# ruc-aimc-lab/LAFF

Hardware: AMD Instinct MI355X
Metric: text-video cosine pairs/sec (higher is better)
Workload: dtype f32 towers (FC on fp16 hi/lo split x3 MFMA) + fp16 similarity

## Files before the change

### laff_amd/build.py

```python
import os
import subprocess
import sys
from concurrent.futures import ThreadPoolExecutor

HERE = os.path.dirname(os.path.abspath(__file__))
CSRC = os.path.join(HERE, 'csrc')
LIBDIR = os.path.join(HERE, 'lib')
LIB = os.path.join(LIBDIR, 'liblaff_hip.so')
SOURCES = ['gemm_nt.hip', 'sim_strip.hip', 'fc_strip.hip', 'fc_concat.hip', 'fuse.hip', 'fuse_bwd.hip', 'frame_bwd.hip', 'fc_bwd.hip', 'optim.hip', 'rank.hip', 'loss.hip', 'loss_dsl.hip', 'gru.hip', 'clip.hip', 'clip_image.hip', 'frame_prep.hip', 'bert.hip', 'netvlad.hip', 'rerank.hip', 'sim_hist.hip', 'comm.hip', 'api.hip']
HEADERS = [os.path.join(CSRC, 'kernels.h'), os.path.join(CSRC, 'clip_core.h'), os.path.join(CSRC, 'exact_cos.h'), os.path.join(CSRC, 'strip_util.h'), os.path.join(CSRC, 'wave_reduce.h'), os.path.join(os.path.dirname(HERE), 'include', 'laff_hip.h')]
ARCH = 'gfx950'
FLAGS = ['-O3', '-std=c++20', '-fPIC', '--offload-arch=' + ARCH, '-fno-gpu-rdc', '-Wall', '-Wno-unused-function']


def hipcc():
    for c in (os.environ.get('HIPCC'), '/opt/rocm/bin/hipcc', 'hipcc'):
        if c and (os.path.isabs(c) and os.path.exists(c) or not os.path.isabs(c)):
            return c
    raise RuntimeError('hipcc not found')


def _stale(target, deps):
    if not os.path.exists(target):
        return True
# ... 43 lines not shown
```

### laff_amd/csrc/api.hip

```cpp
#include <hip/hip_runtime.h>

#include <algorithm>
#include <climits>
#include <cmath>
#include <cstdarg>
#include <cstdio>
#include <cstdlib>
#include <cstring>
#include <string>
#include <vector>

#include "kernels.h"

constexpr int METRIC_SLOTS = 33;

struct laff_ctx {
    int device;
    hipStream_t stream;
    double* d_metrics = nullptr;
    unsigned metrics_slot = 0;
    double* h_metrics = nullptr;
    char* d_mscratch = nullptr;
};

// ... 115 lines not shown
    return LAFF_OK;
}

}

extern "C" {

int laff_abi_version(void) { return LAFF_ABI_VERSION; }

const char* laff_last_error(void) { return g_err.c_str(); }

int laff_ctx_create(int device, void* hip_stream, laff_ctx** out) {
    if (!out) return fail(LAFF_E_ARG, "laff_ctx_create: null out");
    auto knob = [](const char* name, int dflt) { const char* e = getenv(name); return e ? atoi(e) : dflt; };
    laff::g_strip_mode = knob("LAFF_STRIP", 1);
    int n = 0;
    HIP_TRY(hipGetDeviceCount(&n));
    if (device < 0 || device >= n) return fail(LAFF_E_ARG, "laff_ctx_create: device %d out of range (%d devices)", device, n);
    hipDeviceProp_t prop;
    HIP_TRY(hipGetDeviceProperties(&prop, device));
    if (strncmp(prop.gcnArchName, "gfx950", 6) != 0)
        return fail(LAFF_E_UNSUPPORTED, "laff_ctx_create: device %d is %s; this library is built for gfx950 only", device,
                    prop.gcnArchName);
    if (prop.multiProcessorCount > 0) laff::g_num_cus = prop.multiProcessorCount;
    laff_ctx* c = new laff_ctx();
    c->device = device;
    c->stream = static_cast<hipStream_t>(hip_stream);
    *out = c;
    return LAFF_OK;
}
// ... 2061 lines not shown
```

### laff_amd/csrc/fc_strip.hip

```cpp
#include <hip/hip_runtime.h>
#include <stdint.h>

#include <algorithm>
#include <cstdlib>
#include <vector>

#include "kernels.h"
#include "strip_util.h"

namespace laff {

namespace {

using namespace su;

typedef __attribute__((address_space(1))) unsigned gu32;

constexpr int FR = FC_STRIP_ROWS;
constexpr int SLOT = 32 * 1024;
constexpr int PLANE = 16 * 1024;
constexpr int RING = 4;
constexpr int PIECES = 8;
constexpr int XB_OFF = RING * SLOT;
constexpr int SMEM = XB_OFF + SLOT;
// ... 576 lines not shown
        const float b = bias ? bias[n] : 0.f, g = bn_scale ? bn_scale[n] : 1.f, t = bn_shift ? bn_shift[n] : 0.f;
        float4 c;
        if (act == LAFF_ACT_TANH) c = make_float4(cs * 2.885390081777927f, b * 2.885390081777927f, -2.f * g, g + t);
        else if (act == LAFF_ACT_SIGMOID) c = make_float4(cs * -1.4426950408889634f, b * -1.4426950408889634f, g, t);
        else if (act == LAFF_ACT_RELU) c = make_float4(cs, b, g, t);
        else c = make_float4(cs * g, fmaf(b, g, t), 0.f, 0.f);
        *(float4*)(vec + 4 * (size_t)n) = c;
    }
}

size_t fc_strip_image_bytes(int D) { return (size_t)(D / 32) * (2 * SLOT) + (size_t)D * 16; }
size_t fc_strip_vec_offset(int D) { return (size_t)(D / 32) * (2 * SLOT); }

hipError_t launch_fc_strip_pack(const float* W, int ldw, const float* bias, const float* bn_scale, const float* bn_shift, int D, int act,
                                void* img, hipStream_t st) {
    hipLaunchKernelGGL(fc_strip_pack_kernel, dim3((unsigned)D), dim3(256), 0, st, W, ldw, bias, bn_scale, bn_shift, D, act,
                       (_Float16*)img, (float*)((char*)img + fc_strip_vec_offset(D)));
    return hipGetLastError();
}

hipError_t launch_fc_strip(FcStripArgs& a, int act, hipStream_t st) {
    long U = 0;
    for (int i = 0; i < a.count; ++i) {
        a.p[i].unit0 = (int)U;
        U += (long)((a.p[i].N + FR - 1) / FR) * a.nblk;
    }
    if (U == 0) return hipSuccess;
    if (U >= (1l << 31)) return hipErrorInvalidValue;
    a.total_units = (int)U;
    a.trace = nullptr;
#ifdef LAFF_FCS_TRACE
    if (const char* e = getenv("LAFF_GEMM_TRACE_PTR")) a.trace = (unsigned long long*)strtoull(e, nullptr, 0);
#endif
    const int G = (int)std::min<long>(std::min(g_num_cus, STRIP_MAX_WG), U);
    a.nranges = G;
    for (int b = 0; b < G; ++b) a.range_of_wg[b] = (unsigned short)((G % 8 == 0) ? (b % 8) * (G / 8) + b / 8 : b);
#define LAFF_FCS_LAUNCH(K)                                                                                                    \
    do {                                                                                                                      \
        static unsigned long long attr_done = 0;                                                                              \
        if (hipError_t e = smem_attr_once(attr_done, fc_strip_kernel<K>, SMEM); e != hipSuccess) return e;                    \
        hipLaunchKernelGGL((fc_strip_kernel<K>), dim3((unsigned)G), dim3(256), SMEM, st, a);                                  \
    } while (0)
    if (act == LAFF_ACT_TANH || act == LAFF_ACT_SIGMOID) LAFF_FCS_LAUNCH(ACT_EXP);
    else if (act == LAFF_ACT_RELU) LAFF_FCS_LAUNCH(ACT_RELU);
    else LAFF_FCS_LAUNCH(ACT_LIN);
#undef LAFF_FCS_LAUNCH
    return hipGetLastError();
}

}
```

### laff_amd/csrc/kernels.h

```cpp
#pragma once
#include <hip/hip_runtime.h>
#include <stdint.h>

#include "../../include/laff_hip.h"

namespace laff {

template <typename K>
static inline hipError_t smem_attr_once(unsigned long long& done, K kernel, int smem) {
    int dev = 0;
    hipError_t e = hipGetDevice(&dev);
    if (e != hipSuccess) return e;
    const unsigned long long bit = 1ull << (dev & 63);
    if (__atomic_load_n(&done, __ATOMIC_ACQUIRE) & bit) return hipSuccess;
    if (smem > 64 * 1024) {
        e = hipFuncSetAttribute((const void*)kernel, hipFuncAttributeMaxDynamicSharedMemorySize, smem);
        if (e != hipSuccess) return e;
    }
    __atomic_fetch_or(&done, bit, __ATOMIC_ACQ_REL);
    return hipSuccess;
}

enum { GEMM_F32 = 0, GEMM_F16 = 1, GEMM_BF16 = 2 };

// ... 76 lines not shown
};
struct FcStripArgs {
    int count;
    int nblk;
    int nranges;
    int total_units;
    unsigned long long* trace;
    FcStripProblem p[MAX_GROUP];
    unsigned short range_of_wg[STRIP_MAX_WG];
};
size_t fc_strip_image_bytes(int D);
size_t fc_strip_vec_offset(int D);
hipError_t launch_fc_strip_pack(const float* W, int ldw, const float* bias, const float* bn_scale, const float* bn_shift, int D, int act,
                                void* img, hipStream_t st);
hipError_t launch_fc_strip(FcStripArgs& a, int act, hipStream_t st);

constexpr int CONCAT_MAX_SEG = 8;
constexpr int CONCAT_MAX_GROUP = 4;
struct ConcatDense {
    const float* X;
    int ldx, dk, c0;
    int fast;
};
struct ConcatSparse {
    const int* indptr;
    const int* indices;
    const float* values;
    const float* wt;
    int ldwt, dk;
};
// ... 423 lines not shown
```

### laff_amd/model/model.py

```python
import numpy as np

import torch
import torch.nn as nn
import torch.nn.functional as F

from .. import loss as _loss
from .. import ops
from .Attention import Attention_1, JustAverage, Multi_head_MyApply_Attention

device = torch.device('cuda')
float16 = False
FC_PRECISION = 'fp32'


def _row_chunks(pending, limit_bytes=1 << 31):
    out = []
    for q in pending:
        x = q['x']
        if not torch.is_tensor(x) or x.layout != torch.strided or x.dim() != 2:
            out.append(q)
            continue
        n, k = x.shape
        row_bytes = 4 * max(x.stride(0) if n > 1 else k, (k + 63) // 64 * 64)
        if n * row_bytes < limit_bytes:
# ... 211 lines not shown
        return out

    def weight_split(self):
        if FC_PRECISION != 'fp16x3':
            return None
        w = self.fc1.weight
        key = (w.data_ptr(), w._version)
        if getattr(self, '_w_split', None) is None or self._w_split[0] != key:
            self._w_split = (key, ops.split_rows(w.detach()))
        return self._w_split[1]

    def strip_weights(self):
        scale, shift = self.bn_affine(None)
        w, b = self.fc1.weight, self.fc1.bias
        key = (w.data_ptr(), w._version, None if b is None else (b.data_ptr(), b._version),
               None if self.bn1 is None else self._bn_cache[0], self.activation_name)
        if getattr(self, '_w_strip', None) is None or self._w_strip[0] != key:
            self._w_strip = (key, ops.fc_strip_pack(w.detach(), None if b is None else b.detach(), scale, shift, self.activation_name))
        return self._w_strip[1]

    def _forward_train(self, x, heads=1, extra_shift=None):
        if self.fc1 is None:
            raise NotImplementedError('training mode: a TransformNet without fc (fc=False%s) has no differentiable path; apply its '
                                      'BatchNorm upstream as a torch op' % (', tiled over %d heads' % heads if heads > 1 else ''))
        if x.layout != torch.strided:
            raise NotImplementedError('training mode: a sparse (CSR) input has no backward (laff_fc_gather_act_bn is inference only)')
        if extra_shift is not None:
            raise NotImplementedError('training mode: extra_shift (the expert embedding) is not differentiable here; add it upstream '
                                      'as a torch op')
        y = _FcActFn.apply(x, self.fc1.weight, self.fc1.bias, self.activation_name)
        if self.dropout_p is not None:
# ... 717 lines not shown
```

### laff_amd/ops.py

```python
import ctypes as C

import numpy as np
import torch

from . import _lib
from ._lib import (ACT, GRU_POOLING, ATT_JUST_AVERAGE, ATT_L2NORM_EACH_HEAD, ATT_MUL, ATT_NO_SPLIT_HEAD, ATT_WITH_AVE, PREC,
                   FcProblem, FcSplitProblem, FcStripProblem, Plane, check, FcFusedProblem, RankSide, FcConcatProblem, FcConcatSegment,
                   FcLaunch, FcShape, RerankProblem)

__all__ = ['sim_hist', 'rerank_workspace_bytes', 'rerank_run', 'rerank_tkb', 'frame_preprocess', 'frame_desc_device', 'netvlad_workspace_bytes', 'netvlad_encode', 'bert_workspace_bytes', 'bert_encode', 'clip_pack_weight', 'clip_workspace_bytes', 'clip_encode', 'gru_pack_whh', 'gru_workspace_bytes', 'gru_encode', 'rank_resolve_metrics', 'rank_prepare', 'rank_prepare_text', 'rank_band_video', 'rank_export_pairs', 'rank_resolve_list', 'sim_gemm_banded', 'rank_resolve', 'exact_ranks', 'RankState', 'topk_rows', 'topk_from_operands', 'alloc_scores', 'frame_fuse_grouped', 'fc_act_bn_fused_grouped', 'fused_split_eligible', 'fc_strip_pack', 'fc_strip_eligible', 'fc_act_bn_strip_grouped', 'StripWeights', 'margin_loss', 'dsl_loss', 'margin_loss_scores', 'fc_gather_act_bn', 'fc_act_bn', 'fc_act_bn_grouped', 'fc_act_bn_split_grouped', 'split_rows', 'row_dot_gt', 'rank_metrics_async', 'fuse', 'fuse_backward', 'fc_backward', 'fc_backward_plan', 'optim_plan', 'optim_last_launches', 'grad_sqnorm', 'grad_scale', 'optim_step', 'frame_fuse', 'frame_fuse_backward', 'frame_fuse_backward_plan', 'pack_rows', 'sim_gemm', 'sim_gemm_route', 'SIM_ROUTES', 'fc_route', 'FC_ROUTES', 'FcRoute', 'gather_gt', 'rank_count', 'v2t_count', 'v2t_count_exact', 'reset_contexts', 'FusedPrepare', 'fused_prepare_eligible',
           'rank_metrics', 'attention_flags', 'PREC', 'default_prescale']

_ctx = {}

profiler = None


def _call(name, fn, *args):
    if profiler is None:
        check(fn(*args))
    else:
        profiler.begin(name)
        check(fn(*args))
        rep = getattr(profiler, 'repeat', None)
        if rep is not None:
            for _ in range(rep(name) - 1):
                check(fn(*args))
        profiler.end(name)


def _context(device):
    idx = device.index if device.index is not None else torch.cuda.current_device()
    lib = _lib.load()
    if idx not in _ctx:
        h = C.c_void_p()
        check(lib.laff_ctx_create(idx, None, C.byref(h)))
        _ctx[idx] = h
    h = _ctx[idx]
    check(lib.laff_ctx_set_stream(h, C.c_void_p(torch.cuda.current_stream(idx).cuda_stream)))
    return lib, h


def stamp(slots, i):
    lib, h = _context(slots.device)
    check(lib.laff_stamp(h, C.c_void_p(slots.data_ptr() + 8 * int(i))))


def wall_clock_khz(device):
    lib, h = _context(device)
    khz = C.c_int()
    check(lib.laff_wall_clock_khz(h, C.byref(khz)))
    return int(khz.value)
# ... 606 lines not shown
    check(lib.laff_fc_route(h, _FC_FAMILIES[family], arr, n, kind, launch_of, launches, cap, C.byref(nl)))
    out = []
    for j in range(nl.value):
        l = launches[j]
        if l.kernel >= len(FC_ROUTES):
            raise RuntimeError('laff_fc_route: kernel %d is not an FC route' % l.kernel)
        out.append(dict(kernel=FC_ROUTES[l.kernel], problems=[i for i in range(n) if launch_of[i] == j], tiles=int(l.tiles),
                        nbig=int(l.nbig), quarters=int(l.quarters)))
        assert len(out[-1]['problems']) == l.count
    return FcRoute([kind[i] if kind[i] >= 0 else None for i in range(n)], [launch_of[i] if launch_of[i] >= 0 else None for i in range(n)],
                   out)


class StripWeights:

    def __init__(self, img, D, K, act):
        self.img, self.D, self.K, self.act = img, D, K, act


def fc_strip_pack(weight, bias=None, bn_scale=None, bn_shift=None, activation=None):
    w, ldw = _rows(weight, 'weight')
    D, K = w.shape
    lib, h = _context(w.device)
    nbytes = C.c_size_t()
    check(lib.laff_fc_strip_pack_bytes(D, K, C.byref(nbytes)))
    vecs = _fc_vectors(dict(bias=bias, bn_scale=bn_scale, bn_shift=bn_shift), D)
    img = torch.empty((nbytes.value,), device=w.device, dtype=torch.uint8)
    _call('fc_strip_pack', lib.laff_fc_strip_pack, h, _ptr(w), ldw, *vecs, D, K, ACT[activation], _ptr(img))
    return StripWeights(img, D, K, ACT[activation])


def fc_strip_eligible(x, D):
    return (torch.is_tensor(x) and x.is_cuda and x.layout == torch.strided and x.dtype == torch.float32 and x.dim() == 2 and
            x.shape[1] == 512 and (x.shape[0] == 0 or (x.stride(1) == 1 and (x.stride(0) % 4 == 0 or x.shape[0] == 1) and
                                                       x.data_ptr() % 16 == 0)) and D % 32 == 0 and D >= 32)


def fc_act_bn_strip_grouped(problems):
    if not problems:
        return []
    n = len(problems)
    arr = (FcStripProblem * n)()
    outs = []
    dev = problems[0]['strip'].img.device
    for i, q in enumerate(problems):
        x, ldx = _rows(q['x'], 'x')
        sw = q['strip']
        if not fc_strip_eligible(x, sw.D):
            raise ValueError('problem %d is not eligible for the strip form (see fc_strip_eligible)' % i)
        out = q.get('out')
        if out is None:
            out = torch.empty((x.shape[0], sw.D), device=dev, dtype=torch.float32)
        y, ldy = _rows(out, 'out')
        arr[i] = FcStripProblem(x.data_ptr(), max(ldx, 512), x.shape[0], sw.img.data_ptr(), sw.D, sw.act, y.data_ptr(), ldy)
        outs.append(out)
    lib, h = _context(dev)
    _call('fc_act_bn', lib.laff_fc_act_bn_strip_grouped, h, arr, n)
    return outs


def _out_buffer(t, shape, device, name):
    if t is None:
        return torch.empty(shape, device=device, dtype=torch.float32)
    _dev(t, name)
    if tuple(t.shape) != tuple(shape) or not t.is_contiguous() or t.device != device:
        raise ValueError('%s must be a contiguous fp32 %s tensor on %s, got %s' % (name, tuple(shape), device, tuple(t.shape)))
    return t


def fuse(planes, H, d, w, b, gw, flags, return_weights=False, packed_precision=None, l2norm_planes=False, rank_side=None, out=None,
         weights_out=None, packed_out=None):
# ... 992 lines not shown
```

Baseline: 428.4 billion.

## Add 16x16x32 MFMA variant of the FC strip kernel and make it default

Adds a new FC strip kernel built on v_mfma_f32_16x16x32_f16 with its own weight packing layout. It keeps X fragments resident in AGPRs and interleaves a compile-time-scheduled epilogue behind the MFMAs of each column block. An env knob selects it (default 16) or the old 32x32 path, and the Python side tags packed images with the MFMA mode to prevent mismatches. The aim is better overlap of epilogue and loads with matrix work, at the cost of a large, hand-scheduled inline-asm kernel.

Result: faster. 435.9 billion, median of 6 (+1.7%).

```diff
diff --git a/laff_amd/build.py b/laff_amd/build.py
--- a/laff_amd/build.py
+++ b/laff_amd/build.py
@@ -7,7 +7,7 @@
 CSRC = os.path.join(HERE, 'csrc')
 LIBDIR = os.path.join(HERE, 'lib')
 LIB = os.path.join(LIBDIR, 'liblaff_hip.so')
-SOURCES = ['gemm_nt.hip', 'sim_strip.hip', 'fc_strip.hip', 'fc_concat.hip', 'fuse.hip', 'fuse_bwd.hip', 'frame_bwd.hip', 'fc_bwd.hip', 'optim.hip', 'rank.hip', 'loss.hip', 'loss_dsl.hip', 'gru.hip', 'clip.hip', 'clip_image.hip', 'frame_prep.hip', 'bert.hip', 'netvlad.hip', 'rerank.hip', 'sim_hist.hip', 'comm.hip', 'api.hip']
+SOURCES = ['gemm_nt.hip', 'sim_strip.hip', 'fc_strip.hip', 'fc_strip16.hip', 'fc_concat.hip', 'fuse.hip', 'fuse_bwd.hip', 'frame_bwd.hip', 'fc_bwd.hip', 'optim.hip', 'rank.hip', 'loss.hip', 'loss_dsl.hip', 'gru.hip', 'clip.hip', 'clip_image.hip', 'frame_prep.hip', 'bert.hip', 'netvlad.hip', 'rerank.hip', 'sim_hist.hip', 'comm.hip', 'api.hip']
 HEADERS = [os.path.join(CSRC, 'kernels.h'), os.path.join(CSRC, 'clip_core.h'), os.path.join(CSRC, 'exact_cos.h'), os.path.join(CSRC, 'strip_util.h'), os.path.join(CSRC, 'wave_reduce.h'), os.path.join(os.path.dirname(HERE), 'include', 'laff_hip.h')]
 ARCH = 'gfx950'
 FLAGS = ['-O3', '-std=c++20', '-fPIC', '--offload-arch=' + ARCH, '-fno-gpu-rdc', '-Wall', '-Wno-unused-function']
diff --git a/laff_amd/csrc/api.hip b/laff_amd/csrc/api.hip
--- a/laff_amd/csrc/api.hip
+++ b/laff_amd/csrc/api.hip
@@ -153,6 +153,7 @@
     if (!out) return fail(LAFF_E_ARG, "laff_ctx_create: null out");
     auto knob = [](const char* name, int dflt) { const char* e = getenv(name); return e ? atoi(e) : dflt; };
     laff::g_strip_mode = knob("LAFF_STRIP", 1);
+    laff::g_fc_strip_mfma = knob("LAFF_FC_STRIP_MFMA", 16) == 32 ? 32 : 16;
     int n = 0;
     HIP_TRY(hipGetDeviceCount(&n));
     if (device < 0 || device >= n) return fail(LAFF_E_ARG, "laff_ctx_create: device %d out of range (%d devices)", device, n);
diff --git a/laff_amd/csrc/fc_strip.hip b/laff_amd/csrc/fc_strip.hip
--- a/laff_amd/csrc/fc_strip.hip
+++ b/laff_amd/csrc/fc_strip.hip
@@ -614,6 +614,7 @@
 
 hipError_t launch_fc_strip_pack(const float* W, int ldw, const float* bias, const float* bn_scale, const float* bn_shift, int D, int act,
                                 void* img, hipStream_t st) {
+    if (g_fc_strip_mfma != 32) return launch_fc_strip16_pack(W, ldw, bias, bn_scale, bn_shift, D, act, img, st);
     hipLaunchKernelGGL(fc_strip_pack_kernel, dim3((unsigned)D), dim3(256), 0, st, W, ldw, bias, bn_scale, bn_shift, D, act,
                        (_Float16*)img, (float*)((char*)img + fc_strip_vec_offset(D)));
     return hipGetLastError();
@@ -635,6 +636,7 @@
     const int G = (int)std::min<long>(std::min(g_num_cus, STRIP_MAX_WG), U);
     a.nranges = G;
     for (int b = 0; b < G; ++b) a.range_of_wg[b] = (unsigned short)((G % 8 == 0) ? (b % 8) * (G / 8) + b / 8 : b);
+    if (g_fc_strip_mfma != 32) return launch_fc_strip16(a, act, st);
 #define LAFF_FCS_LAUNCH(K)                                                                                                    \
     do {                                                                                                                      \
         static unsigned long long attr_done = 0;                                                                              \
diff --git a/laff_amd/csrc/fc_strip16.hip b/laff_amd/csrc/fc_strip16.hip
--- /dev/null
+++ b/laff_amd/csrc/fc_strip16.hip
@@ -0,0 +1,652 @@
+#include <hip/hip_runtime.h>
+#include <stdint.h>
+
+#include <algorithm>
+#include <cstdlib>
+#include <vector>
+
+#include "kernels.h"
+#include "strip_util.h"
+#include "wave_reduce.h"
+
+namespace laff {
+
+namespace {
+
+using namespace su;
+
+typedef __attribute__((address_space(1))) unsigned gu32;
+typedef float f32x2 __attribute__((ext_vector_type(2)));
+
+constexpr int FR = FC_STRIP_ROWS;
+constexpr int SLOT = 32 * 1024;
+constexpr int PLANE = 16 * 1024;
+constexpr int RING = 4;
+constexpr int PIECES = 8;
+constexpr int XB_OFF = RING * SLOT;
+constexpr int SMEM = XB_OFF + SLOT;
+static_assert(SMEM <= 160 * 1024, "LDS budget");
+
+constexpr int FD = 6;
+constexpr int NSETS = 8;
+static_assert(32 % NSETS == 0 && FD < NSETS - 1 && FD % 2 == 0, "the set of a fragment must not depend on the block");
+constexpr int BAR_J = 16 - FD;
+constexpr int NSLOT = 192;
+
+struct AgprHold { u32x4 q[64]; };
+#define HOLD16(OP, h, b)                                                                                                                  \
+    OP(h.q[b], h.q[b + 1], h.q[b + 2], h.q[b + 3], h.q[b + 4], h.q[b + 5], h.q[b + 6], h.q[b + 7], h.q[b + 8], h.q[b + 9], h.q[b + 10], h.q[b + 11], \
+       h.q[b + 12], h.q[b + 13], h.q[b + 14], h.q[b + 15])
+#define HOLD_DEF(x0, x1, x2, x3, x4, x5, x6, x7, x8, x9, xa, xb, xc, xd, xe, xf)                                                            \
+    asm volatile("" : "=a"(x0), "=a"(x1), "=a"(x2), "=a"(x3), "=a"(x4), "=a"(x5), "=a"(x6), "=a"(x7), "=a"(x8), "=a"(x9), "=a"(xa), "=a"(xb), \
+                 "=a"(xc), "=a"(xd), "=a"(xe), "=a"(xf))
+#define HOLD_USE(x0, x1, x2, x3, x4, x5, x6, x7, x8, x9, xa, xb, xc, xd, xe, xf)                                                            \
+    asm volatile("" ::"a"(x0), "a"(x1), "a"(x2), "a"(x3), "a"(x4), "a"(x5), "a"(x6), "a"(x7), "a"(x8), "a"(x9), "a"(xa), "a"(xb), "a"(xc),   \
+                 "a"(xd), "a"(xe), "a"(xf))
+__device__ __forceinline__ void agpr_hold_begin(AgprHold& h) { HOLD16(HOLD_DEF, h, 0); HOLD16(HOLD_DEF, h, 16); HOLD16(HOLD_DEF, h, 32); HOLD16(HOLD_DEF, h, 48); }
+__device__ __forceinline__ void agpr_hold_end(AgprHold& h) { HOLD16(HOLD_USE, h, 0); HOLD16(HOLD_USE, h, 16); HOLD16(HOLD_USE, h, 32); HOLD16(HOLD_USE, h, 48); }
+
+template <int R, int OFF>
+__device__ __forceinline__ void agpr_load4(const void* p) {
+    asm volatile("global_load_dwordx4 a[%c1:%c2], %0, off offset:%c3" ::"v"(p), "n"(R), "n"(R + 3), "n"(OFF) : "memory");
+}
+template <int R>
+__device__ __forceinline__ float agpr_read() {
+    float x;
+    asm volatile("v_accvgpr_read_b32 %0, a[%c1]" : "=v"(x) : "n"(R));
+    return x;
+}
+template <int R>
+__device__ __forceinline__ void agpr_write(unsigned x) { asm volatile("v_accvgpr_write_b32 a[%c1], %0" ::"v"(x), "n"(R)); }
+
+template <int R, bool FIRST>
+__device__ __forceinline__ void mfma_strip(f32x4& acc, const u32x4& wfrag) {
+    if constexpr (FIRST) asm volatile("v_mfma_f32_16x16x32_f16 %0, a[%c2:%c3], %1, 0" : "=v"(acc) : "v"(wfrag), "n"(R), "n"(R + 3));
+    else asm volatile("v_mfma_f32_16x16x32_f16 %0, a[%c2:%c3], %1, %0" : "+v"(acc) : "v"(wfrag), "n"(R), "n"(R + 3));
+}
+
+template <int IMM>
+__device__ __forceinline__ void lds_read128(u32x4& d, unsigned addr) {
+    asm volatile("ds_read_b128 %0, %1 offset:%2" : "=v"(d) : "v"(addr), "n"(IMM));
+}
+
+template <int LDSOFF>
+__device__ __forceinline__ void dma_piece(unsigned voff, u32x4 rsrc, unsigned soff, unsigned m0base) {
+    asm volatile("s_add_i32 m0, %3, %4\n\ts_nop 0\n\tbuffer_load_dwordx4 %0, %1, %2 offen lds"
+                 ::"v"(voff), "s"(rsrc), "s"(soff), "s"(m0base), "n"(LDSOFF) : "memory", "scc");
+}
+
+template <int LDSOFF>
+__device__ __forceinline__ void dma_rows(unsigned voff, unsigned long long base, unsigned m0base) {
+    asm volatile("s_add_i32 m0, %2, %3\n\ts_nop 0\n\tglobal_load_lds_dwordx4 %0, %1 "
+                 ::"v"(voff), "s"(base), "s"(m0base), "n"(LDSOFF) : "memory", "scc");
+}
+template <int R, int IMM>
+__device__ __forceinline__ void lds_to_agpr(unsigned addr) {
+    asm volatile("ds_read_b128 a[%c1:%c2], %0 offset:%c3" ::"v"(addr), "n"(R), "n"(R + 3), "n"(IMM) : "memory");
+}
+template <typename T>
+__device__ __forceinline__ void pin_v(T& x) { asm volatile("" : "+v"(x)); }
+template <int ROWMUL>
+__device__ __forceinline__ void store_row(unsigned& tmp, f32x2 data, unsigned voff0, unsigned ldy4, u32x4 rsrc, unsigned soff) {
+    asm volatile("v_mad_u32_u24 %0, %3, %4, %2\n\tbuffer_store_dwordx2 %1, %0, %5, %6 offen nt"
+                 : "=&v"(tmp) : "v"(data), "v"(voff0), "s"(ldy4), "n"(ROWMUL), "s"(rsrc), "s"(soff) : "memory");
+}
+
+__device__ __forceinline__ int split_exponent(float m) {
+    const int be = (int)((__float_as_uint(m) >> 23) & 0xffu);
+    if (!(m > 0.f) || be == 0xff) return 0;
+    return max(be - 127, -100);
+}
+__device__ __forceinline__ float pow2f(int e) { return __uint_as_float((unsigned)(e + 127) << 23); }
+template <int R>
+__device__ __forceinline__ void stash_chunk(const u32x4& q0, const u32x4& q1, float& m0, float& m1) {
+    asm volatile("v_max3_f32 %0, |%2|, |%3|, %0\n\tv_max3_f32 %1, |%4|, |%5|, %1\n\tv_max3_f32 %0, |%6|, |%7|, %0\n\tv_max3_f32 %1, |%8|, |%9|, %1\n\t"
+                 "v_accvgpr_write_b32 a[%c10+0], %2\n\tv_accvgpr_write_b32 a[%c10+1], %3\n\tv_accvgpr_write_b32 a[%c10+2], %4\n\t"
+                 "v_accvgpr_write_b32 a[%c10+3], %5\n\tv_accvgpr_write_b32 a[%c10+4], %6\n\tv_accvgpr_write_b32 a[%c10+5], %7\n\t"
+                 "v_accvgpr_write_b32 a[%c10+6], %8\n\tv_accvgpr_write_b32 a[%c10+7], %9"
+                 : "+v"(m0), "+v"(m1) : "v"(q0.x), "v"(q0.y), "v"(q0.z), "v"(q0.w), "v"(q1.x), "v"(q1.y), "v"(q1.z), "v"(q1.w), "n"(R));
+}
+template <int R>
+__device__ __forceinline__ void convert_chunk_inplace(float s) {
+    float x0, x1, x2, x3, x4, x5, x6, x7;
+    unsigned h0, h1, h2, h3, l0, l1, l2, l3;
+    asm volatile(
+        "v_accvgpr_read_b32 %0, a[%c17+0]\n\tv_accvgpr_read_b32 %1, a[%c17+1]\n\tv_accvgpr_read_b32 %2, a[%c17+2]\n\tv_accvgpr_read_b32 %3, a[%c17+3]\n\t"
+        "v_accvgpr_read_b32 %4, a[%c17+4]\n\tv_accvgpr_read_b32 %5, a[%c17+5]\n\tv_accvgpr_read_b32 %6, a[%c17+6]\n\tv_accvgpr_read_b32 %7, a[%c17+7]\n\t"
+        "v_fma_mixlo_f16 %8, %0, %16, 0\n\tv_fma_mixlo_f16 %9, %2, %16, 0\n\tv_fma_mixlo_f16 %10, %4, %16, 0\n\tv_fma_mixlo_f16 %11, %6, %16, 0\n\t"
+        "v_fma_mixhi_f16 %8, %1, %16, 0\n\tv_fma_mixhi_f16 %9, %3, %16, 0\n\tv_fma_mixhi_f16 %10, %5, %16, 0\n\tv_fma_mixhi_f16 %11, %7, %16, 0\n\t"
+        "v_fma_mix_f32 %0, %0, %16, -%8 op_sel:[0,0,0] op_sel_hi:[0,0,1]\n\tv_fma_mix_f32 %2, %2, %16, -%9 op_sel:[0,0,0] op_sel_hi:[0,0,1]\n\t"
+        "v_fma_mix_f32 %4, %4, %16, -%10 op_sel:[0,0,0] op_sel_hi:[0,0,1]\n\tv_fma_mix_f32 %6, %6, %16, -%11 op_sel:[0,0,0] op_sel_hi:[0,0,1]\n\t"
+        "v_fma_mix_f32 %1, %1, %16, -%8 op_sel:[0,0,1] op_sel_hi:[0,0,1]\n\tv_fma_mix_f32 %3, %3, %16, -%9 op_sel:[0,0,1] op_sel_hi:[0,0,1]\n\t"
+        "v_fma_mix_f32 %5, %5, %16, -%10 op_sel:[0,0,1] op_sel_hi:[0,0,1]\n\tv_fma_mix_f32 %7, %7, %16, -%11 op_sel:[0,0,1] op_sel_hi:[0,0,1]\n\t"
+        "v_accvgpr_write_b32 a[%c17+0], %8\n\tv_accvgpr_write_b32 a[%c17+1], %9\n\tv_accvgpr_write_b32 a[%c17+2], %10\n\tv_accvgpr_write_b32 a[%c17+3], %11\n\t"
+        "v_cvt_pk_f16_f32 %12, %0, %1\n\tv_cvt_pk_f16_f32 %13, %2, %3\n\tv_cvt_pk_f16_f32 %14, %4, %5\n\tv_cvt_pk_f16_f32 %15, %6, %7\n\t"
+        "v_accvgpr_write_b32 a[%c17+4], %12\n\tv_accvgpr_write_b32 a[%c17+5], %13\n\tv_accvgpr_write_b32 a[%c17+6], %14\n\tv_accvgpr_write_b32 a[%c17+7], %15"
+        : "=&v"(x0), "=&v"(x1), "=&v"(x2), "=&v"(x3), "=&v"(x4), "=&v"(x5), "=&v"(x6), "=&v"(x7), "=&v"(h0), "=&v"(h1), "=&v"(h2), "=&v"(h3),
+          "=&v"(l0), "=&v"(l1), "=&v"(l2), "=&v"(l3)
+        : "v"(s), "n"(R));
+}
+__device__ __forceinline__ void absmax3(float& m, float x, float y) { asm volatile("v_max3_f32 %0, |%1|, |%2|, %0" : "+v"(m) : "v"(x), "v"(y)); }
+__device__ __forceinline__ void split_pair(float& x0, float& x1, float s, unsigned& hi, unsigned& lo) {
+    asm volatile("v_fma_mixlo_f16 %0, %1, %2, 0" : "=v"(hi) : "v"(x0), "v"(s));
+    asm volatile("v_fma_mixhi_f16 %0, %1, %2, 0" : "+v"(hi) : "v"(x1), "v"(s));
+    asm volatile("v_fma_mix_f32 %0, %0, %1, -%2 op_sel:[0,0,0] op_sel_hi:[0,0,1]" : "+v"(x0) : "v"(s), "v"(hi));
+    asm volatile("v_fma_mix_f32 %0, %0, %1, -%2 op_sel:[0,0,1] op_sel_hi:[0,0,1]" : "+v"(x1) : "v"(s), "v"(hi));
+    asm volatile("v_cvt_pk_f16_f32 %0, %1, %2" : "=v"(lo) : "v"(x0), "v"(x1));
+}
+
+enum : unsigned char { OP_WAITCV = 0, OP_MUL, OP_FMA1, OP_EXP, OP_ADD1, OP_RCP, OP_MAX, OP_FMA2, OP_ST };
+enum { ACT_LIN = 0, ACT_RELU = 1, ACT_EXP = 2 };
+struct EpiOp { unsigned char kind, elem; };
+struct EpiStream { EpiOp op[160]; int n; };
+constexpr int op_cost(unsigned char k) { return (k == OP_EXP || k == OP_RCP || k == OP_ST) ? 8 : (k == OP_WAITCV ? 0 : 4); }
+constexpr int SLOT_CYCLES = 8;
+
+template <int ACTK>
+constexpr EpiStream make_stream() {
+    EpiStream s{};
+    s.n = 0;
+    auto push = [&](unsigned char k, int e) { s.op[s.n++] = EpiOp{k, (unsigned char)e}; };
+    push(OP_WAITCV, 0);
+    for (int g = 0; g < 4; ++g) {
+        auto stage = [&](unsigned char k) { for (int e = 0; e < 4; ++e) push(k, 4 * g + e); };
+        stage(OP_MUL);
+        stage(OP_FMA1);
+        if (ACTK == ACT_EXP) { stage(OP_EXP); stage(OP_ADD1); stage(OP_RCP); stage(OP_FMA2); }
+        if (ACTK == ACT_RELU) { stage(OP_MAX); stage(OP_FMA2); }
+        push(OP_ST, 4 * g);
+        push(OP_ST, 4 * g + 2);
+    }
+    return s;
+}
+constexpr int DRAIN_STORES = 8;
+
+constexpr int slot_piece(int sg) {
+    const int F = (sg % 96) / 6, m = sg % 6;
+    if (m == 2 && F >= BAR_J) return F - BAR_J;
+    if (m == 4 && F == BAR_J + 1) return 6;
+    if (m == 4 && F == BAR_J + 4) return 7;
+    return -1;
+}
+constexpr bool slot_cvload(int sg) { return sg == 1; }
+struct Plan {
+    short begin[NSLOT + 1];
+    short vm_bar[2];
+    short vm_cv;
+    short st_half[2];
+    bool fits;
+};
+template <int ACTK>
+constexpr Plan make_plan() {
+    Plan p{};
+    const EpiStream st = make_stream<ACTK>();
+    int usable = 0, total = 0;
+    auto ok = [](int sg) { return sg >= 6 && sg % 6 != 0 && slot_piece(sg) < 0; };
+    for (int sg = 0; sg < NSLOT; ++sg) usable += ok(sg) ? 1 : 0;
+    for (int i = 0; i < st.n; ++i) total += op_cost(st.op[i].kind);
+    usable -= 6;
+    int at = 0, k = 0, spent = 0;
+    for (int sg = 0; sg < NSLOT; ++sg) {
+        p.begin[sg] = (short)at;
+        if (!ok(sg)) continue;
+        ++k;
+        const int target = (int)(((long)k * total + usable - 1) / usable);
+        int here = 0;
+        while (at < st.n && spent < target) {
+            const int c = op_cost(st.op[at].kind);
+            if (here + c > SLOT_CYCLES) break;
+            here += c; spent += c; ++at;
+        }
+    }
+    p.begin[NSLOT] = (short)at;
+    p.fits = at == st.n;
+    int vm_n = 0, last_piece[3][2] = {}, cv_ord[3] = {}, bar_at[3][2] = {}, waitcv_at[3] = {};
+    for (int blk = 0; blk < 3; ++blk)
+        for (int sg = 0; sg < NSLOT; ++sg) {
+            const int H = sg / 96, F = (sg % 96) / 6, m = sg % 6;
+            if (F == BAR_J && m == 0) bar_at[blk][H] = vm_n;
+            if (slot_cvload(sg)) { vm_n += 2; cv_ord[blk] = vm_n; }
+            if (slot_piece(sg) >= 0) { ++vm_n; last_piece[blk][H] = vm_n; }
+            for (int i = p.begin[sg]; i < p.begin[sg + 1]; ++i) {
+                if (st.op[i].kind == OP_WAITCV) waitcv_at[blk] = vm_n;
+                if (st.op[i].kind == OP_ST) { ++vm_n; if (blk == 2) ++p.st_half[H]; }
+            }
+        }
+    auto clamp = [](int c) { return c < 0 ? 0 : (c > 63 ? 63 : c); };
+    for (int H = 0; H < 2; ++H) p.vm_bar[H] = (short)clamp(bar_at[2][H] - last_piece[1][H]);
+    p.vm_cv = (short)clamp(waitcv_at[2] - cv_ord[1]);
+    return p;
+}
+
+}
+
+template <int ACTK>
+__global__ __launch_bounds__(256, 1) void fc_strip16_kernel(const FcStripArgs a) {
+    extern __shared__ __attribute__((aligned(1024))) char smem[];
+    AgprHold hold;
+    agpr_hold_begin(hold);
+    const int tid = threadIdx.x, lane = tid & 63;
+    const int wave = __builtin_amdgcn_readfirstlane(tid >> 6);
+    const int n15 = lane & 15, g4 = lane >> 4;
+    const unsigned lds0 = (unsigned)(size_t)((__attribute__((address_space(3))) char*)smem);
+
+    const int nblk = pin_s(a.nblk), count = pin_s(a.count);
+    const int nranges = pin_s(a.nranges);
+    const long U = (long)pin_s((unsigned)a.total_units);
+    const int myrange = a.range_of_wg[blockIdx.x];
+    int u0 = pin_s((int)(U * myrange / nranges));
+    const int u1 = pin_s((int)(U * (myrange + 1) / nranges));
+    const unsigned img_bytes = (unsigned)nblk * (2u * SLOT);
+
+    constexpr Plan PLAN = make_plan<ACTK>();
+    constexpr EpiStream STREAM = make_stream<ACTK>();
+    static_assert(PLAN.fits, "the epilogue stream does not fit behind the MFMAs of one column block");
+
+    unsigned lane16 = (unsigned)lane * 16u;
+    asm volatile("" : "+v"(lane16));
+    const unsigned xa0 = lds0 + lane16, xa1 = lds0 + lane16 + 2u * SLOT;
+    const unsigned wslot = (unsigned)wave * (PIECES * 1024u);
+    const unsigned ldsw = pin_s(lds0 + wslot);
+    const unsigned cvoff = (unsigned)n15 * 32u;
+    int pre_base = -1;
+    const unsigned m0_keep = m0_get();
+#ifdef LAFF_FCS_TRACE
+    unsigned long long* const trc = a.trace ? a.trace + (size_t)blockIdx.x * 80 : nullptr;
+    int trc_seg = 0;
+#define STAMP(i) do { if (trc && tid == 0 && trc_seg < 8) trc[8 * trc_seg + (i)] = __builtin_readcyclecounter(); } while (0)
+#else
+#define STAMP(i) do {} while (0)
+#endif
+
+    while (u0 < u1) {
+        int p = 0;
+        while (p + 1 < count && u0 >= a.p[p + 1].unit0) ++p;
+        p = __builtin_amdgcn_readfirstlane(p);
+        const int ul = u0 - a.p[p].unit0;
+        const int strip = __builtin_amdgcn_readfirstlane(ul / nblk);
+        const int blk0 = __builtin_amdgcn_readfirstlane(ul - strip * nblk);
+        const int n = __builtin_amdgcn_readfirstlane(std::min(nblk - blk0, u1 - u0));
+        u0 += n;
+        STAMP(0);
+#ifdef LAFF_FCS_TRACE
+        if (trc && tid == 0 && trc_seg < 8) trc[64 + trc_seg] = (unsigned long long)n;
+#endif
+        auto xoff = [&](int p_, int strip_, unsigned (&xv)[8]) {
+            const int N_ = a.p[p_].N, ldx_ = a.p[p_].ldx, r0_ = strip_ * FR;
+            int ln = lane;
+            asm volatile("" : "+v"(ln));
+#pragma unroll
+            for (int t = 0; t < 8; ++t) {
+                const int rw = 4 * t + (ln >> 4);
+                const int r = std::min(r0_ + wave * 32 + rw, N_ - 1) - r0_;
+                xv[t] = (unsigned)r * (unsigned)ldx_ * 4u + ((((unsigned)ln & 15u) ^ ((unsigned)rw & 15u)) << 4);
+            }
+        };
+        const bool has_next = u0 < u1 && n >= 2;
+        int p2 = p, strip2 = strip;
+        if (has_next) {
+            p2 = 0;
+            while (p2 + 1 < count && u0 >= a.p[p2 + 1].unit0) ++p2;
+            p2 = __builtin_amdgcn_readfirstlane(p2);
+            strip2 = __builtin_amdgcn_readfirstlane((u0 - a.p[p2].unit0) / nblk);
+        }
+        unsigned xvn[8];
+        xoff(p2, strip2, xvn);
+#pragma unroll
+        for (int t = 0; t < 8; ++t) asm volatile("" : "+v"(xvn[t]));
+        const u32x4 rsrcXn = rebased_rsrc((unsigned long long)a.p[p2].X + (unsigned long long)(strip2 * FR) * (unsigned)a.p[p2].ldx * 4ull,
+                                          (unsigned long long)FR * (unsigned)a.p[p2].ldx * 4ull, 0ull);
+        const int N = pin_s(a.p[p].N), ldx = pin_s(a.p[p].ldx), ldy = pin_s(a.p[p].ldy);
+        const unsigned long long pX = pin_s((unsigned long long)a.p[p].X), pW = pin_s((unsigned long long)a.p[p].img);
+        const unsigned long long pVec = pin_s((unsigned long long)a.p[p].vec), pY = pin_s((unsigned long long)a.p[p].Y);
+        const int row0 = strip * FR;
+
+        f32x4 acc[2][2][2];
+        u32x4 fr[NSETS][2];
+        float rs[8];
+        f32x2 tt[4] = {{0, 0}, {0, 0}, {0, 0}, {0, 0}};
+        unsigned ta[4] = {0, 0, 0, 0};
+        f32x4 cv[2][2] = {{{0, 0, 0, 0}, {0, 0, 0, 0}}, {{0, 0, 0, 0}, {0, 0, 0, 0}}};
+
+        int e_row[2] = {0, 0};
+        {
+            const unsigned long long xbase = pX + (unsigned long long)row0 * (unsigned)ldx * 4ull;
+            unsigned xv[8];
+            xoff(p, strip, xv);
+            const bool pre = pre_base >= 0;
+            const int base = pre ? pre_base : 0;
+            unsigned XA[8];
+            {
+                unsigned ln = (unsigned)lane;
+                asm volatile("" : "+v"(ln));
+#pragma unroll
+                for (int j = 0; j < 8; ++j)
+                    XA[j] = ((ln & 15u) + 16u * (unsigned)((j >> 1) & 1)) * 256u + ((((unsigned)(8 * (j >> 2) + 4 * (j & 1)) + (ln >> 4)) ^ (ln & 15u)) << 4);
+            }
+            auto buf_of = [&](int e) __attribute__((always_inline)) {
+                const int ring = pre ? (e < 3 ? e : (e == 4 ? 3 : e - 5)) : (e < 4 ? e : e - 5);
+                const bool x = pre ? (e == 3 || e == 7) : e == 4;
+                return ldsw + (unsigned)(x ? RING : ((ring + base) & 3)) * (unsigned)SLOT;
+            };
+            auto issue_round = [&](auto EC) __attribute__((always_inline)) {
+                constexpr int e = decltype(EC)::value;
+                const unsigned long long ebase = xbase + (unsigned long long)(e * 256);
+                const unsigned b = pin_s(buf_of(e));
+                static_for<0, 8>([&](auto TC) __attribute__((always_inline)) {
+                    constexpr int t = decltype(TC)::value;
+                    dma_rows<t * 1024>(xv[t], ebase, b);
+                });
+            };
+            float m0[2] = {0.f, 0.f}, m1[2] = {0.f, 0.f};
+            u32x4 rq[8];
+            auto read_round = [&](auto EC) __attribute__((always_inline)) {
+                constexpr int e = decltype(EC)::value;
+                const unsigned b = buf_of(e);
+                static_for<0, 8>([&](auto JC) __attribute__((always_inline)) { constexpr int j = decltype(JC)::value; lds_read128<0>(rq[j], XA[j] + b); });
+                wait_lgkm<0>();
+                static_for<0, 8>([&](auto IC) __attribute__((always_inline)) { pin_v(rq[decltype(IC)::value]); });
+            };
+            auto stash_round = [&](auto EC) __attribute__((always_inline)) {
+                constexpr int e = decltype(EC)::value;
+                static_for<0, 4>([&](auto CC) __attribute__((always_inline)) {
+                    constexpr int cc = decltype(CC)::value;
+                    stash_chunk<8 * (4 * e + cc)>(rq[2 * cc], rq[2 * cc + 1], m0[cc & 1], m1[cc & 1]);
+                });
+            };
+            using E0 = std::integral_constant<int, 0>; using E1 = std::integral_constant<int, 1>; using E2 = std::integral_constant<int, 2>;
+            using E3 = std::integral_constant<int, 3>; using E4 = std::integral_constant<int, 4>; using E5 = std::integral_constant<int, 5>;
+            using E6 = std::integral_constant<int, 6>; using E7 = std::integral_constant<int, 7>;
+            if (!pre) {
+                issue_round(E0{}); issue_round(E1{}); issue_round(E2{}); issue_round(E3{}); issue_round(E4{});
+                wait_vm<32>(); read_round(E0{}); issue_round(E5{}); stash_round(E0{});
+                wait_vm<32>(); read_round(E1{}); issue_round(E6{}); stash_round(E1{});
+                wait_vm<32>(); read_round(E2{}); issue_round(E7{}); stash_round(E2{});
+                wait_vm<32>(); read_round(E3{}); stash_round(E3{});
+                wait_vm<24>(); read_round(E4{}); stash_round(E4{});
+            } else {
+                constexpr int DR = DRAIN_STORES, S1 = PLAN.st_half[1];
+                wait_vm<(10 + 8 + DR) + 8 + DR>(); read_round(E0{}); issue_round(E5{}); stash_round(E0{});
+                wait_vm<(8 + S1) + 8 + DR + 8>(); read_round(E1{}); issue_round(E6{}); stash_round(E1{});
+                read_round(E3{}); issue_round(E7{}); stash_round(E3{});
+                wait_vm<8 + DR + 24>(); read_round(E2{}); stash_round(E2{});
+                wait_vm<24>(); read_round(E4{}); stash_round(E4{});
+            }
+            wait_vm<16>(); read_round(E5{}); stash_round(E5{});
+            wait_vm<8>(); read_round(E6{}); stash_round(E6{});
+            wait_vm<0>(); read_round(E7{}); stash_round(E7{});
+#pragma unroll
+            for (int t = 0; t < 2; ++t) {
+                float m = fmaxf(m0[t], m1[t]);
+                m = wave_step32<16>(m, [](float x, float y) { return fmaxf(x, y); });
+                m = wave_step32<32>(m, [](float x, float y) { return fmaxf(x, y); });
+                e_row[t] = split_exponent(m);
+            }
+            pre_base = has_next ? ((n & 1) ? 2 : 0) : -1;
+        }
+        __builtin_amdgcn_s_barrier();
+        asm volatile("" ::: "memory");
+        STAMP(1);
+
+        const u32x4 rsrcW = rebased_rsrc(pW, img_bytes, wslot);
+        unsigned soffW = (unsigned)blk0 * (2u * SLOT);
+        static_for<0, 3>([&](auto SC) __attribute__((always_inline)) {
+            constexpr int s = decltype(SC)::value;
+            static_for<0, PIECES>([&](auto PC) __attribute__((always_inline)) {
+                constexpr int P = decltype(PC)::value;
+                dma_piece<s * SLOT + P * 1024>(lane16 + (unsigned)(P * 1024), rsrcW, std::min(soffW, img_bytes - SLOT), ldsw);
+            });
+            soffW += SLOT;
+        });
+
+        STAMP(2);
+        {
+            const float s0 = pow2f(9 - e_row[0]), s1 = pow2f(9 - e_row[1]);
+            asm volatile("s_nop 1" ::: "memory");
+            static_for<0, 32>([&](auto GC) __attribute__((always_inline)) { convert_chunk_inplace<8 * decltype(GC)::value>((decltype(GC)::value & 1) ? s1 : s0); });
+        }
+        asm volatile("s_nop 3" ::: "memory");
+        STAMP(3);
+        {
+            const float mine0 = pow2f(e_row[0] - 9), mine1 = pow2f(e_row[1] - 9);
+#pragma unroll
+            for (int i = 0; i < 8; ++i) rs[i] = __shfl((i >> 2) ? mine1 : mine0, 4 * g4 + (i & 3));
+        }
+        const unsigned ldy4 = (unsigned)ldy * 4u;
+        unsigned voff0 = ((unsigned)(wave * 32 + 4 * g4) * (unsigned)ldy + 2u * (unsigned)n15) * 4u;
+        const u32x4 rsrcY = rebased_rsrc(pY + (unsigned long long)row0 * (unsigned)ldy * 4ull,
+                                         ((unsigned long long)(std::min(FR, N - row0) - 1) * (unsigned)ldy + (unsigned)(nblk * 32)) * 4ull, 0ull);
+        const u32x4 rsrcNone = {0u, 0u, 0u, 0x00020000u};
+        const u32x4 rsrcV = rebased_rsrc(pVec, (unsigned long long)nblk * 512ull, 0ull);
+
+        asm volatile("s_waitcnt vmcnt(0) lgkmcnt(0)" ::: "memory");
+#pragma unroll
+        for (int i = 0; i < 8; ++i) asm volatile("" : "+v"(rs[i]));
+        asm volatile("" : "+v"(voff0));
+        __builtin_amdgcn_s_barrier();
+        asm volatile("" ::: "memory");
+        STAMP(4);
+        static_for<0, FD>([&](auto JC) __attribute__((always_inline)) {
+            constexpr int j = decltype(JC)::value;
+            lds_read128<j * 1024>(fr[j][0], xa0);
+            lds_read128<PLANE + j * 1024>(fr[j][1], xa0);
+        });
+
+        u32x4 rsrcYe = rsrcNone;
+        unsigned soffY = 0u;
+        using I0 = std::integral_constant<int, 0>;
+        using I1 = std::integral_constant<int, 1>;
+        using I2 = std::integral_constant<int, 2>;
+        using IM1 = std::integral_constant<int, -1>;
+        auto epi_item = [&](auto QC, auto IC, auto DRAIN) __attribute__((always_inline)) {
+            constexpr int Q = decltype(QC)::value;
+            constexpr EpiOp op = STREAM.op[decltype(IC)::value];
+            constexpr int i = op.elem, u = i & 1, e = (i >> 1) & 3, t = i >> 3, k = (i >> 1) & 3;
+            if constexpr (op.kind == OP_WAITCV) {
+                if constexpr (decltype(DRAIN)::value >= 0) wait_vm<16 + DRAIN_STORES + decltype(DRAIN)::value>(); else wait_vm<PLAN.vm_cv>();
+                asm volatile("" : "+v"(cv[Q][0]), "+v"(cv[Q][1]));
+            } else if constexpr (op.kind == OP_MUL) {
+                asm volatile("v_mul_f32 %0, %1, %2" : "=v"(tt[k][u]) : "v"(acc[Q][t][u][e]), "v"(rs[4 * t + e]));
+            } else if constexpr (op.kind == OP_FMA1) {
+                asm volatile("v_fma_f32 %0, %0, %1, %2" : "+v"(tt[k][u]) : "v"(cv[Q][u].x), "v"(cv[Q][u].y));
+            } else if constexpr (op.kind == OP_EXP) {
+                asm volatile("v_exp_f32 %0, %0" : "+v"(tt[k][u]));
+            } else if constexpr (op.kind == OP_ADD1) {
+                asm volatile("v_add_f32 %0, 1.0, %0" : "+v"(tt[k][u]));
+            } else if constexpr (op.kind == OP_RCP) {
+                asm volatile("v_rcp_f32 %0, %0" : "+v"(tt[k][u]));
+            } else if constexpr (op.kind == OP_MAX) {
+                asm volatile("v_max_f32 %0, 0, %0" : "+v"(tt[k][u]));
+            } else if constexpr (op.kind == OP_FMA2) {
+                asm volatile("v_fma_f32 %0, %0, %1, %2" : "+v"(tt[k][u]) : "v"(cv[Q][u].z), "v"(cv[Q][u].w));
+            } else if constexpr (op.kind == OP_ST) {
+                store_row<16 * t + e>(ta[k], tt[k], voff0, ldy4, rsrcYe, soffY);
+            }
+        };
+
+        auto body = [&](auto PARC, auto HC, auto XRC, int blk) __attribute__((always_inline)) {
+            constexpr int PAR = decltype(PARC)::value, H = decltype(HC)::value, Q = PAR ^ 1;
+            constexpr int XR = decltype(XRC)::value;
+            constexpr int RSLOT = 2 * PAR + H;
+            constexpr int NSLOT_R = (RSLOT + 1) & 3;
+            constexpr int DSLOT = (RSLOT + 3) & 3;
+            const unsigned soff_here = std::min(soffW, img_bytes - SLOT);
+            soffW += SLOT;
+            if constexpr (H == 0) soffY = (unsigned)(blk - 1) * 128u;
+            static_for<0, 16>([&](auto FC) __attribute__((always_inline)) {
+                constexpr int F = decltype(FC)::value;
+                constexpr int G = 16 * H + F;
+                if constexpr (F == BAR_J) {
+                    if constexpr (XR != 2) wait_vm<PLAN.vm_bar[H]>();
+                    __builtin_amdgcn_s_barrier();
+                    asm volatile("" ::: "memory");
+                }
+                if constexpr (F % 2 == 0) wait_lgkm<2 * (FD - 2)>();
+                __builtin_amdgcn_sched_barrier(0);
+                static_for<0, 6>([&](auto MC) __attribute__((always_inline)) {
+                    constexpr int m = decltype(MC)::value, SG = 96 * H + 6 * F + m;
+                    constexpr int s12 = SG % 12, JG = SG / 12, M = s12 / 4, u = (s12 % 4) / 2, t = s12 & 1;
+                    constexpr int R = 16 * JG + 8 * t, GS = (2 * JG + u) % NSETS;
+                    if constexpr (M == 0) mfma_strip<R + 4, (JG == 0)>(acc[PAR][t][u], fr[GS][0]);
+                    else if constexpr (M == 1) mfma_strip<R, false>(acc[PAR][t][u], fr[GS][1]);
+                    else mfma_strip<R, false>(acc[PAR][t][u], fr[GS][0]);
+                    __builtin_amdgcn_sched_barrier(0);
+                    if constexpr (m == 0) {
+                        constexpr int FN = F + FD;
+                        constexpr int RS = FN < 16 ? RSLOT : NSLOT_R, FF = FN & 15, GN = (G + FD) % NSETS;
+                        constexpr int OFFS = (RS & 1) * SLOT + FF * 1024;
+                        if constexpr (RS < 2) {
+                            lds_read128<OFFS>(fr[GN][0], xa0);
+                            lds_read128<OFFS + PLANE>(fr[GN][1], xa0);
+                        } else {
+                            lds_read128<OFFS>(fr[GN][0], xa1);
+                            lds_read128<OFFS + PLANE>(fr[GN][1], xa1);
+                        }
+                    }
+                    if constexpr (slot_cvload(SG)) {
+                        const unsigned so = (unsigned)blk * 512u;
+                        asm volatile("buffer_load_dwordx4 %0, %2, %3, %4 offen\n\tbuffer_load_dwordx4 %1, %2, %3, %4 offen offset:16"
+                                     : "=&v"(cv[PAR][0]), "=&v"(cv[PAR][1]) : "v"(cvoff), "s"(rsrcV), "s"(so) : "memory");
+                    }
+                    if constexpr (XR == 0 && m == 2 && F < 8) {
+                        dma_piece<XB_OFF + F * 1024>(xvn[F], rsrcXn, 3u * 256u, ldsw);
+                    }
+                    constexpr int dp = slot_piece(SG);
+                    if constexpr (dp >= 0) {
+                        if constexpr (XR >= 0) dma_piece<DSLOT * SLOT + dp * 1024>(xvn[dp], rsrcXn, (unsigned)(256 * XR), ldsw);
+                        else dma_piece<DSLOT * SLOT + dp * 1024>(lane16 + (unsigned)(dp * 1024), rsrcW, soff_here, ldsw);
+                    }
+                    static_for<PLAN.begin[SG], PLAN.begin[SG + 1]>([&](auto IC) __attribute__((always_inline)) {
+                        __builtin_amdgcn_sched_barrier(0);
+                        epi_item(std::integral_constant<int, Q>{}, IC, IM1{});
+                    });
+                    __builtin_amdgcn_sched_barrier(0);
+                });
+            });
+        };
+
+        auto drain = [&](auto QC, auto EXTRA, int blk) __attribute__((always_inline)) {
+            STAMP(5);
+            mfma_drain_nops();
+            rsrcYe = rsrcY;
+            soffY = (unsigned)blk * 128u;
+            static_for<0, STREAM.n>([&](auto IC) __attribute__((always_inline)) { epi_item(QC, IC, EXTRA); });
+        };
+        auto plain = [&](auto PARC, int b) __attribute__((always_inline)) {
+            body(PARC, I0{}, IM1{}, blk0 + b);
+            body(PARC, I1{}, IM1{}, blk0 + b);
+        };
+        auto tail = [&](auto PARC, int b) __attribute__((always_inline)) {
+            constexpr int P = decltype(PARC)::value;
+            body(PARC, I0{}, IM1{}, blk0 + b);
+            body(PARC, I1{}, I0{}, blk0 + b);
+            rsrcYe = rsrcY;
+            body(std::integral_constant<int, P ^ 1>{}, I0{}, I1{}, blk0 + b + 1);
+            body(std::integral_constant<int, P ^ 1>{}, I1{}, I2{}, blk0 + b + 1);
+            asm volatile("s_waitcnt lgkmcnt(0)" ::: "memory");
+            __builtin_amdgcn_s_barrier();
+            static_for<0, 8>([&](auto TC) __attribute__((always_inline)) {
+                constexpr int t = decltype(TC)::value;
+                dma_piece<(2 * (P ^ 1) + 1) * SLOT + t * 1024>(xvn[t], rsrcXn, 4u * 256u, ldsw);
+            });
+            drain(std::integral_constant<int, P ^ 1>{}, std::integral_constant<int, 8>{}, blk0 + b + 1);
+        };
+#pragma unroll
+        for (int e = 0; e < 4; ++e) acc[1][0][0][e] = acc[1][0][1][e] = acc[1][1][0][e] = acc[1][1][1][e] = 0.0f;
+        {
+            const int m = has_next ? n - 2 : n;
+            int b = 0, par = 0;
+            if (m > 0) {
+#pragma nounroll
+                for (;;) {
+                    plain(I0{}, b);
+                    rsrcYe = rsrcY;
+                    if (++b >= m) { par = 1; break; }
+                    plain(I1{}, b);
+                    if (++b >= m) { par = 0; break; }
+                }
+            }
+            if (has_next) {
+                if (par == 0) tail(I0{}, b); else tail(I1{}, b);
+            } else {
+                if (par == 1) drain(I0{}, I0{}, blk0 + b - 1); else drain(I1{}, I0{}, blk0 + b - 1);
+            }
+        }
+        asm volatile("s_waitcnt lgkmcnt(0)" ::: "memory");
+#pragma unroll
+        for (int s8 = 0; s8 < NSETS; ++s8) asm volatile("" ::"v"(fr[s8][0]), "v"(fr[s8][1]));
+        if (!has_next) __builtin_amdgcn_s_barrier();
+        STAMP(6);
+#ifdef LAFF_FCS_TRACE
+        ++trc_seg;
+#endif
+    }
+    asm volatile("s_waitcnt vmcnt(0)" ::: "memory");
+    m0_set(m0_keep);
+    agpr_hold_end(hold);
+#undef STAMP
+}
+
+__global__ __launch_bounds__(256) void fc_strip16_pack_kernel(const float* __restrict__ W, int ldw, const float* __restrict__ bias,
+                                                              const float* __restrict__ bn_scale, const float* __restrict__ bn_shift, int D,
+                                                              int act, _Float16* __restrict__ img, float* __restrict__ vec) {
+    __shared__ float red[4];
+    const int n = blockIdx.x, tid = threadIdx.x;
+    if (n >= D) return;
+    const float x0 = W[(size_t)n * ldw + tid], x1 = W[(size_t)n * ldw + 256 + tid];
+    float m = fmaxf(fabsf(x0), fabsf(x1));
+#pragma unroll
+    for (int o = 32; o >= 1; o >>= 1) m = fmaxf(m, __shfl_xor(m, o));
+    if ((tid & 63) == 0) red[tid >> 6] = m;
+    __syncthreads();
+    m = fmaxf(fmaxf(red[0], red[1]), fmaxf(red[2], red[3]));
+    const int e = split_exponent(m);
+    const float s = pow2f(9 - e), cs = pow2f(e - 9);
+    const int blk = n >> 5, n15 = (n & 31) >> 1, u = n & 1;
+#pragma unroll
+    for (int t = 0; t < 2; ++t) {
+        const int k = t * 256 + tid;
+        const float x = (t ? x1 : x0) * s;
+        const _Float16 h = (_Float16)x, l = (_Float16)(x - (float)h);
+        const int J = k >> 5, w = k & 31;
+        const int half = J >> 3, Jl = J & 7, g = (w >> 2) & 3, pos = (w & 3) + 4 * (w >> 4);
+        const size_t base = ((size_t)(blk * 2 + half) * 2) * (PLANE / 2);
+        const size_t at = (size_t)((2 * Jl + u) * 64 + 16 * g + n15) * 8 + pos;
+        img[base + at] = h;
+        img[base + PLANE / 2 + at] = l;
+    }
+    if (tid == 0) {
+        const float b = bias ? bias[n] : 0.f, g = bn_scale ? bn_scale[n] : 1.f, t = bn_shift ? bn_shift[n] : 0.f;
+        float4 c;
+        if (act == LAFF_ACT_TANH) c = make_float4(cs * 2.885390081777927f, b * 2.885390081777927f, -2.f * g, g + t);
+        else if (act == LAFF_ACT_SIGMOID) c = make_float4(cs * -1.4426950408889634f, b * -1.4426950408889634f, g, t);
+        else if (act == LAFF_ACT_RELU) c = make_float4(cs, b, g, t);
+        else c = make_float4(cs * g, fmaf(b, g, t), 0.f, 0.f);
+        *(float4*)(vec + 4 * (size_t)n) = c;
+    }
+}
+
+int g_fc_strip_mfma = 16;
+
+hipError_t launch_fc_strip16_pack(const float* W, int ldw, const float* bias, const float* bn_scale, const float* bn_shift, int D, int act,
+                                  void* img, hipStream_t st) {
+    hipLaunchKernelGGL(fc_strip16_pack_kernel, dim3((unsigned)D), dim3(256), 0, st, W, ldw, bias, bn_scale, bn_shift, D, act,
+                       (_Float16*)img, (float*)((char*)img + fc_strip_vec_offset(D)));
+    return hipGetLastError();
+}
+
+hipError_t launch_fc_strip16(const FcStripArgs& a, int act, hipStream_t st) {
+#define LAFF_FCS_LAUNCH(K)                                                                                                    \
+    do {                                                                                                                      \
+        static unsigned long long attr_done = 0;                                                                              \
+        if (hipError_t e = smem_attr_once(attr_done, fc_strip16_kernel<K>, SMEM); e != hipSuccess) return e;                  \
+        hipLaunchKernelGGL((fc_strip16_kernel<K>), dim3((unsigned)a.nranges), dim3(256), SMEM, st, a);                        \
+    } while (0)
+    if (act == LAFF_ACT_TANH || act == LAFF_ACT_SIGMOID) LAFF_FCS_LAUNCH(ACT_EXP);
+    else if (act == LAFF_ACT_RELU) LAFF_FCS_LAUNCH(ACT_RELU);
+    else LAFF_FCS_LAUNCH(ACT_LIN);
+#undef LAFF_FCS_LAUNCH
+    return hipGetLastError();
+}
+
+}
diff --git a/laff_amd/csrc/kernels.h b/laff_amd/csrc/kernels.h
--- a/laff_amd/csrc/kernels.h
+++ b/laff_amd/csrc/kernels.h
@@ -114,6 +114,10 @@
 hipError_t launch_fc_strip_pack(const float* W, int ldw, const float* bias, const float* bn_scale, const float* bn_shift, int D, int act,
                                 void* img, hipStream_t st);
 hipError_t launch_fc_strip(FcStripArgs& a, int act, hipStream_t st);
+extern int g_fc_strip_mfma;
+hipError_t launch_fc_strip16_pack(const float* W, int ldw, const float* bias, const float* bn_scale, const float* bn_shift, int D, int act,
+                                  void* img, hipStream_t st);
+hipError_t launch_fc_strip16(const FcStripArgs& a, int act, hipStream_t st);
 
 constexpr int CONCAT_MAX_SEG = 8;
 constexpr int CONCAT_MAX_GROUP = 4;
diff --git a/laff_amd/model/model.py b/laff_amd/model/model.py
--- a/laff_amd/model/model.py
+++ b/laff_amd/model/model.py
@@ -249,7 +249,7 @@
         scale, shift = self.bn_affine(None)
         w, b = self.fc1.weight, self.fc1.bias
         key = (w.data_ptr(), w._version, None if b is None else (b.data_ptr(), b._version),
-               None if self.bn1 is None else self._bn_cache[0], self.activation_name)
+               None if self.bn1 is None else self._bn_cache[0], self.activation_name, ops.fc_strip_mfma(w.device))
         if getattr(self, '_w_strip', None) is None or self._w_strip[0] != key:
             self._w_strip = (key, ops.fc_strip_pack(w.detach(), None if b is None else b.detach(), scale, shift, self.activation_name))
         return self._w_strip[1]
diff --git a/laff_amd/ops.py b/laff_amd/ops.py
--- a/laff_amd/ops.py
+++ b/laff_amd/ops.py
@@ -1,4 +1,6 @@
 import ctypes as C
+import os
+import re
 
 import numpy as np
 import torch
@@ -12,6 +14,7 @@
            'rank_metrics', 'attention_flags', 'PREC', 'default_prescale']
 
 _ctx = {}
+_fc_strip_mfma = 16
 
 profiler = None
 
@@ -29,6 +32,16 @@
         profiler.end(name)
 
 
+def _atoi(text):
+    m = re.match(r'\s*[+-]?\d+', text)
+    return int(m.group(0)) if m else 0
+
+
+def fc_strip_mfma(device):
+    _context(device)
+    return _fc_strip_mfma
+
+
 def _context(device):
     idx = device.index if device.index is not None else torch.cuda.current_device()
     lib = _lib.load()
@@ -36,6 +49,8 @@
         h = C.c_void_p()
         check(lib.laff_ctx_create(idx, None, C.byref(h)))
         _ctx[idx] = h
+        global _fc_strip_mfma
+        _fc_strip_mfma = 32 if _atoi(os.environ.get('LAFF_FC_STRIP_MFMA', '16')) == 32 else 16
     h = _ctx[idx]
     check(lib.laff_ctx_set_stream(h, C.c_void_p(torch.cuda.current_stream(idx).cuda_stream)))
     return lib, h
@@ -672,8 +687,8 @@
 
 class StripWeights:
 
-    def __init__(self, img, D, K, act):
-        self.img, self.D, self.K, self.act = img, D, K, act
+    def __init__(self, img, D, K, act, mfma):
+        self.img, self.D, self.K, self.act, self.mfma = img, D, K, act, mfma
 
 
 def fc_strip_pack(weight, bias=None, bn_scale=None, bn_shift=None, activation=None):
@@ -685,7 +700,7 @@
     vecs = _fc_vectors(dict(bias=bias, bn_scale=bn_scale, bn_shift=bn_shift), D)
     img = torch.empty((nbytes.value,), device=w.device, dtype=torch.uint8)
     _call('fc_strip_pack', lib.laff_fc_strip_pack, h, _ptr(w), ldw, *vecs, D, K, ACT[activation], _ptr(img))
-    return StripWeights(img, D, K, ACT[activation])
+    return StripWeights(img, D, K, ACT[activation], _fc_strip_mfma)
 
 
 def fc_strip_eligible(x, D):
@@ -713,6 +728,10 @@
         arr[i] = FcStripProblem(x.data_ptr(), max(ldx, 512), x.shape[0], sw.img.data_ptr(), sw.D, sw.act, y.data_ptr(), ldy)
         outs.append(out)
     lib, h = _context(dev)
+    for i, q in enumerate(problems):
+        if q['strip'].mfma != _fc_strip_mfma:
+            raise ValueError('problem %d: its image was packed under LAFF_FC_STRIP_MFMA=%d, the context runs %d: pack it again'
+                             % (i, q['strip'].mfma, _fc_strip_mfma))
     _call('fc_act_bn', lib.laff_fc_act_bn_strip_grouped, h, arr, n)
     return outs
 
```
